# BrandonHanx/TextReID

Hardware: AMD Instinct MI355X
Metric: image-text pairs/sec (train), CLIP-RN50 + BiGRU MoCo step, bs128/GPU (higher is better)
Workload: dtype f32; 1 GPU; configs[1]: CLIP-RN50 + GRU, bs128/GPU, 384x128 images, 64-token captions, MoCo queue 8192, fp32, 1xMI355X; random-init weights, synthetic inputs resident in HBM; global_batch=128, parallelism=dp1, optimizer=Adam (fused multi-tensor), step_launch=eager launches, four streams (chosen by the probe over the recorded step)

## Files before the change

textreid_amd/csrc/gemm_p16.hip:

```cpp

#include <algorithm>
#include <mutex>
#include <type_traits>

#include "split_common.h"

namespace trid {

constexpr int P16_BK = 32;
constexpr int A_CONV_S2 = 3;

constexpr int p16_lds_bytes(int BM, int BN, int NW, int STAGES) {
    const int st = STAGES * (BM + BN) * 128;
    return (NW == 12 && BM * BN * 4 > st) ? BM * BN * 4 : st;
}

template <int N>
__device__ __forceinline__ void wait_vmcnt() {
    asm volatile("s_waitcnt vmcnt(%0)" ::"n"(N) : "memory");
}

__device__ __forceinline__ void dma16(const __amdgpu_buffer_rsrc_t& rs, uint4* lds_base, unsigned voffset, unsigned soffset) {
    typedef __attribute__((address_space(3))) void* lds_ptr;
    __builtin_amdgcn_raw_ptr_buffer_load_lds(rs, (lds_ptr)lds_base, 16, voffset, soffset, 0, 0);
}

typedef int v4i_t __attribute__((ext_vector_type(4)));
__device__ __forceinline__ v4i_t raw_rsrc(const void* base, unsigned bytes) {
    const unsigned long long b = (unsigned long long)(uintptr_t)base;
    v4i_t r;
    r[0] = __builtin_amdgcn_readfirstlane((int)(unsigned)b);
    r[1] = __builtin_amdgcn_readfirstlane((int)(unsigned)(b >> 32) & 0xffff);
    r[2] = __builtin_amdgcn_readfirstlane((int)bytes);
    r[3] = 0x00020000;
    return r;
}
__device__ __forceinline__ void dma16_asm(const v4i_t& rs, unsigned lds_byte_addr, unsigned voffset, unsigned soffset) {
    asm volatile("s_mov_b32 m0, %0\n\ts_nop 0\n\tbuffer_load_dwordx4 %1, %2, %3 offen lds" ::"s"(__builtin_amdgcn_readfirstlane(lds_byte_addr)), "v"(voffset), "s"(rs), "s"(__builtin_amdgcn_readfirstlane(soffset)) : "memory", "m0");
}

template <int AMODE, int BM, int BN, int WM, int WN, int STAGES, int PL, bool PP = false, int SP = 0>
__global__ __launch_bounds__(WM* WN * 64, (WM * WN == 4 && STAGES == 2) ? 2 : (WM * WN == 8 && (BM + BN) * 128 * STAGES <= 80 * 1024 ? 4 : ((WM * WN == 6 || WM * WN == 12) ? 3 : 2))) void gemm_p16_kernel(GemmParams p) {
    constexpr int NW = WM * WN;
    constexpr bool CONV = AMODE == A_CONV || AMODE == A_CONV_S2, S2 = AMODE == A_CONV_S2;
    constexpr int BKE = PL == 2 ? 32 : 64;
    constexpr int EB = PL == 2 ? 4 : 2;
    constexpr int TM = BM / (32 * WM), TN = BN / (32 * WN);
    constexpr int A_CH = BM / 8, B_CH = BN / 8;
    constexpr int A_PW = (A_CH + NW - 1) / NW, B_PW = (B_CH + NW - 1) / NW;
    constexpr int PER_TILE = A_PW + B_PW;
    constexpr int STAGE_SLOTS = (BM + BN) * 8;
    extern __shared__ __attribute__((aligned(16))) uint4 smem[];

    const float scaleA = (PL == 2 && p.a_amax != nullptr) ? f16_scale_of(*p.a_amax) : 1.f;
    const float scaleB = (PL == 2 && p.b_amax != nullptr) ? f16_scale_of(*p.b_amax) : 1.f;
    float ev_bound = 0.f, ev_rinv = 1.f;
    unsigned ev_seen = 0;
    if (p.c_fmt == 1) {
        ev_bound = eval_out_bound(p.ev);
        ev_rinv = p.res16 != nullptr ? 1.f / f16_scale_of(*p.res16_amax) : 1.f;
        if (p.ev.out_tmax != nullptr) ev_seen = __hip_atomic_load(reinterpret_cast<const unsigned*>(p.ev.out_tmax), __ATOMIC_RELAXED, __HIP_MEMORY_SCOPE_AGENT);
    }

    const int tid = threadIdx.x;
    const int lane = tid & 63;
    const int wave = __builtin_amdgcn_readfirstlane(tid >> 6);
    const int wm = wave / WN, wn = wave % WN;
    const int khalf = lane >> 5;

    const uint32_t nwg = (uint32_t)p.mblocks * (uint32_t)p.nblocks;
    const uint32_t lid = xcd_remap(blockIdx.x, nwg);
    const int mb = lid / p.nblocks, nb = lid % p.nblocks;
    const int m0 = mb * BM, n0 = nb * BN;
    const int z = blockIdx.z;
    const int bz = z / p.splits, sz = z % p.splits;
    const int kt_begin = sz * (p.k_chunk / BKE);
    const int kt_end = min(p.K / BKE, kt_begin + p.k_chunk / BKE);
    const int nk = kt_end - kt_begin;

    const char* A = reinterpret_cast<const char*>(p.A) + (long long)bz * p.sA * EB;
    const char* Bp = reinterpret_cast<const char*>(p.B) + (long long)bz * p.sB * EB;
    float* __restrict__ C = p.C + (long long)bz * p.sC + (long long)sz * p.sSplit;
    const float* __restrict__ bias = p.bias ? p.bias + (long long)bz * p.sBias : nullptr;

    constexpr unsigned OOB = 0x80000000u;
    const long long a_ld_bytes = (CONV ? (long long)p.Cin : p.lda) * EB;
    const long long a_rows = CONV ? (S2 ? (long long)(p.M / (p.RH * p.RW)) * p.H * p.W : (long long)p.M) + 2 * p.W + 2 : p.M;
    const char* a_base = (CONV) ? A - (long long)(p.W + 1) * a_ld_bytes : A;
    const __amdgpu_buffer_rsrc_t rsA = __builtin_amdgcn_make_buffer_rsrc((void*)a_base, 0, (unsigned)(a_rows * a_ld_bytes), 0x00020000);
    const __amdgpu_buffer_rsrc_t rsB = __builtin_amdgcn_make_buffer_rsrc((void*)Bp, 0, (unsigned)((long long)p.N * p.ldb * EB), 0x00020000);

    unsigned voA[A_PW], voB[B_PW], amask[A_PW];
#pragma unroll
    for (int j = 0; j < A_PW; ++j) {
        const int c = j * NW + wave;
        const int r = 8 * c + (lane >> 3);
        const int s = (lane & 7) ^ ((r >> 1) & 7);
        const int m = m0 + r;
        voA[j] = (c < A_CH && m < p.M) ? (unsigned)((long long)m * a_ld_bytes + 16 * s) : OOB;
        amask[j] = 0x1ffu;
        if constexpr (S2) {
            const uint32_t mm = m < p.M ? (uint32_t)m : 0u;
            const uint32_t q = fdiv(mm, p.fdW);
            const int x = (int)mm - (int)q * p.RW;
            const uint32_t b = fdiv(q, p.fdH);
            const int y = (int)q - (int)b * p.RH;
            const long long src = ((long long)b * p.H + 2 * y) * p.W + 2 * x;
            voA[j] = (c < A_CH && m < p.M) ? (unsigned)(src * a_ld_bytes + 16 * s) : OOB;
            unsigned mk = 0;
#pragma unroll
            for (int t = 0; t < 9; ++t) {
                const int yy = 2 * y + t / 3 - 1, xx = 2 * x + t % 3 - 1;
                if (yy >= 0 && yy < p.H && xx >= 0 && xx < p.W) mk |= 1u << t;
            }
            amask[j] = mk;
        } else if (CONV) {
            const uint32_t q = fdiv((uint32_t)m, p.fdW);
            const int x = m - (int)q * p.W;
            const uint32_t b = fdiv(q, p.fdH);
            const int y = (int)q - (int)b * p.H;
            unsigned mk = 0;
#pragma unroll
            for (int t = 0; t < 9; ++t) {
                const int yy = y + t / 3 - 1, xx = x + t % 3 - 1;
                if (yy >= 0 && yy < p.H && xx >= 0 && xx < p.W) mk |= 1u << t;
            }
            amask[j] = mk;
        }
    }
#pragma unroll
    for (int j = 0; j < B_PW; ++j) {
        const int c = j * NW + wave;
        const int r = 8 * c + (lane >> 3);
        const int s = (lane & 7) ^ ((r >> 1) & 7);
        const int n = n0 + r;
        voB[j] = (c < B_CH && n < p.N) ? (unsigned)((long long)n * p.ldb * EB + 16 * s) : OOB;
    }
    const int cgroups = (CONV) ? p.Cin / BKE : 1;

    const unsigned smem_base = (unsigned)(uintptr_t)(__attribute__((address_space(3))) void*)smem;
    auto issue = [&](int kt, int stage) {
        uint4* sA = smem + stage * STAGE_SLOTS;
        uint4* sB = sA + BM * 8;
        unsigned soA, soB;
        int tap = 0;
        if (CONV) {
            tap = kt % 9;
            const int cg = kt / 9;
            soA = (unsigned)((((tap / 3) * p.W + (tap % 3)) * (long long)p.Cin * EB) + cg * 128);
            soB = (unsigned)((tap * cgroups + cg) * 128);
        } else {
            soA = soB = (unsigned)(kt * 128);
        }
#pragma unroll
        for (int j = 0; j < A_PW; ++j) {
            const int c = j * NW + wave;
            if (A_CH % NW != 0 && c >= A_CH) break;
            unsigned vo = voA[j];
            if (CONV) vo = ((amask[j] >> tap) & 1u) ? vo : OOB;
            dma16(rsA, sA + c * 64, vo, soA);
        }
#pragma unroll
        for (int j = 0; j < B_PW; ++j) {
            const int c = j * NW + wave;
            if (B_CH % NW != 0 && c >= B_CH) break;
            dma16(rsB, sB + c * 64, voB[j], soB);
        }
    };

    v16f acc[TM][TN];
#pragma unroll
    for (int i = 0; i < TM; ++i)
#pragma unroll
        for (int j = 0; j < TN; ++j)
#pragma unroll
            for (int r = 0; r < 16; ++r) acc[i][j][r] = 0.f;

    const int xs = (lane >> 1) & 7;
    const int a_row = wm * (32 * TM) + (lane & 31);
    const int b_row = wn * (32 * TN) + (lane & 31);

    auto compute = [&](int stage) {
        const uint4* sA = smem + stage * STAGE_SLOTS;
        const uint4* sB = sA + BM * 8;
        if constexpr (PL == 1) {
#pragma unroll
            for (int ks = 0; ks < 4; ++ks) {
                bf16x8 a[TM], b[TN];
                const int s = (2 * ks + khalf) ^ xs;
#pragma unroll
                for (int i = 0; i < TM; ++i) a[i] = __builtin_bit_cast(bf16x8, sA[(a_row + 32 * i) * 8 + s]);
#pragma unroll
                for (int j = 0; j < TN; ++j) b[j] = __builtin_bit_cast(bf16x8, sB[(b_row + 32 * j) * 8 + s]);
#pragma unroll
                for (int i = 0; i < TM; ++i)
#pragma unroll
                    for (int j = 0; j < TN; ++j) acc[i][j] = __builtin_amdgcn_mfma_f32_32x32x16_bf16(a[i], b[j], acc[i][j], 0, 0, 0);
            }
        } else {
#pragma unroll
            for (int ks = 0; ks < 2; ++ks) {
                f16x8 a[2][TM], b[2][TN];
#pragma unroll
                for (int pl = 0; pl < 2; ++pl) {
                    const int s = (4 * pl + 2 * ks + khalf) ^ xs;
#pragma unroll
                    for (int i = 0; i < TM; ++i) a[pl][i] = __builtin_bit_cast(f16x8, sA[(a_row + 32 * i) * 8 + s]);
#pragma unroll
                    for (int j = 0; j < TN; ++j) b[pl][j] = __builtin_bit_cast(f16x8, sB[(b_row + 32 * j) * 8 + s]);
                }
#pragma unroll
                for (int i = 0; i < TM; ++i)
#pragma unroll
                    for (int j = 0; j < TN; ++j) acc[i][j] = __builtin_amdgcn_mfma_f32_32x32x16_f16(a[0][i], b[1][j], acc[i][j], 0, 0, 0);
#pragma unroll
                for (int i = 0; i < TM; ++i)
#pragma unroll
                    for (int j = 0; j < TN; ++j) acc[i][j] = __builtin_amdgcn_mfma_f32_32x32x16_f16(a[1][i], b[0][j], acc[i][j], 0, 0, 0);
#pragma unroll
                for (int i = 0; i < TM; ++i)
#pragma unroll
                    for (int j = 0; j < TN; ++j) acc[i][j] = __builtin_amdgcn_mfma_f32_32x32x16_f16(a[0][i], b[0][j], acc[i][j], 0, 0, 0);
            }
        }
    };

    if constexpr (PP) {
        static_assert(STAGES == 2 && NW % 2 == 0, "ping-pong schedule: two stages, an even number of waves");
        constexpr int NKS = PL == 2 ? 2 : 4, NPL = PL == 2 ? 2 : 1;
        uint4 fa[NKS][NPL][TM], fb[NKS][NPL][TN];
        auto rd = [&](int stage) {
            const uint4* sA = smem + stage * STAGE_SLOTS;
            const uint4* sB = sA + BM * 8;
#pragma unroll
            for (int ks = 0; ks < NKS; ++ks)
#pragma unroll
                for (int pl = 0; pl < NPL; ++pl) {
                    const int s = ((PL == 2 ? 4 * pl : 0) + 2 * ks + khalf) ^ xs;
#pragma unroll
                    for (int i = 0; i < TM; ++i) fa[ks][pl][i] = sA[(a_row + 32 * i) * 8 + s];
#pragma unroll
                    for (int j = 0; j < TN; ++j) fb[ks][pl][j] = sB[(b_row + 32 * j) * 8 + s];
                }
            asm volatile("s_waitcnt lgkmcnt(0)" ::: "memory");
        };
        auto mm = [&]() {
            __builtin_amdgcn_s_setprio(1);
#pragma unroll
            for (int ks = 0; ks < NKS; ++ks) {
                if constexpr (PL == 1) {
#pragma unroll
                    for (int i = 0; i < TM; ++i)
#pragma unroll
                        for (int j = 0; j < TN; ++j)
                            acc[i][j] = __builtin_amdgcn_mfma_f32_32x32x16_bf16(__builtin_bit_cast(bf16x8, fa[ks][0][i]), __builtin_bit_cast(bf16x8, fb[ks][0][j]), acc[i][j], 0, 0, 0);
                } else {
#pragma unroll
                    for (int i = 0; i < TM; ++i)
#pragma unroll
                        for (int j = 0; j < TN; ++j)
                            acc[i][j] = __builtin_amdgcn_mfma_f32_32x32x16_f16(__builtin_bit_cast(f16x8, fa[ks][0][i]), __builtin_bit_cast(f16x8, fb[ks][1][j]), acc[i][j], 0, 0, 0);
#pragma unroll
                    for (int i = 0; i < TM; ++i)
#pragma unroll
                        for (int j = 0; j < TN; ++j)
                            acc[i][j] = __builtin_amdgcn_mfma_f32_32x32x16_f16(__builtin_bit_cast(f16x8, fa[ks][1][i]), __builtin_bit_cast(f16x8, fb[ks][0][j]), acc[i][j], 0, 0, 0);
#pragma unroll
                    for (int i = 0; i < TM; ++i)
// ... 21 lines not shown
                bar();
            }
            bar();
        } else {
            if (1 < nk) issue(kt_begin + 1, 1);
            bar();
            for (int t = 0; t < nk; ++t) {
                rd(t & 1);
                wait_vmcnt<0>();
                bar();
                if (t + 2 < nk) issue(kt_begin + t + 2, t & 1);
                mm();
                bar();
            }
        }
    } else if constexpr (SP != 0) {
        static_assert(STAGES == 2 && PL == 2, "software pipeline: two stages, P16 operands");
        constexpr int NM = 3 * TM * TN;
        const v4i_t rsA_s = raw_rsrc(a_base, (unsigned)(a_rows * a_ld_bytes)), rsB_s = raw_rsrc(Bp, (unsigned)((long long)p.N * p.ldb * EB));
        uint4 f0a[2][TM], f0b[2][TN], f1a[2][TM], f1b[2][TN];
        auto rd = [&](int stage, int ks, uint4 (&fa)[2][TM], uint4 (&fb)[2][TN]) {
            const uint4* sA = smem + stage * STAGE_SLOTS;
            const uint4* sB = sA + BM * 8;
#pragma unroll
            for (int pl = 0; pl < 2; ++pl) {
                const int s = (4 * pl + 2 * ks + khalf) ^ xs;
#pragma unroll
                for (int i = 0; i < TM; ++i) fa[pl][i] = sA[(a_row + 32 * i) * 8 + s];
#pragma unroll
                for (int j = 0; j < TN; ++j) fb[pl][j] = sB[(b_row + 32 * j) * 8 + s];
            }
        };
        auto mm1 = [&](const uint4 (&fa)[2][TM], const uint4 (&fb)[2][TN], int idx) {
            const int pr = idx / (TM * TN), ij = idx % (TM * TN), i = ij / TN, j = ij % TN;
            const int pa = pr == 1 ? 1 : 0, pb = pr == 0 ? 1 : 0;
            acc[i][j] = __builtin_amdgcn_mfma_f32_32x32x16_f16(__builtin_bit_cast(f16x8, fa[pa][i]), __builtin_bit_cast(f16x8, fb[pb][j]), acc[i][j], 0, 0, 0);
        };
        int n_tap = 0, n_dx = 0;
        unsigned n_soA = 0, n_soB = 0, n_rowA = 0, n_cgA = 0;
        const unsigned cin_b = (unsigned)p.Cin * EB, roww_b = (unsigned)p.W * cin_b;
        {
            const int kt = kt_begin;
            if (CONV) {
                n_tap = kt % 9;
                const int cg = kt / 9;
                n_dx = n_tap % 3;
                n_rowA = (unsigned)(n_tap / 3) * roww_b;
                n_cgA = (unsigned)cg * 128u;
                n_soA = n_rowA + (unsigned)n_dx * cin_b + n_cgA;
                n_soB = (unsigned)(n_tap * cgroups + cg) * 128u;
            } else {
                n_soA = n_soB = (unsigned)kt * 128u;
            }
        }
        unsigned c_soA = 0, c_soB = 0;
        int c_tap = 0;
        auto latch = [&]() {
            c_soA = n_soA; c_soB = n_soB; c_tap = n_tap;
        };
        auto advance = [&]() {
            if (CONV) {
                ++n_tap; ++n_dx;
                n_soB += (unsigned)cgroups * 128u;
                if (n_dx == 3) { n_dx = 0; n_rowA += roww_b; }
                if (n_tap == 9) { n_tap = 0; n_rowA = 0; n_cgA += 128u; n_soB = n_soB - 9u * (unsigned)cgroups * 128u + 128u; }
                n_soA = n_rowA + (unsigned)n_dx * cin_b + n_cgA;
            } else {
                n_soA += 128u; n_soB += 128u;
            }
        };
        auto piece = [&](int stage, int q) {
            if (q < A_PW) {
                const int c = q * NW + wave;
                if (A_CH % NW != 0 && c >= A_CH) return;
                unsigned vo = voA[q];
                if (CONV) vo = ((amask[q] >> c_tap) & 1u) ? vo : OOB;
                dma16_asm(rsA_s, smem_base + (unsigned)(stage * STAGE_SLOTS + c * 64) * 16u, vo, c_soA);
            } else {
                const int j = q - A_PW, c = j * NW + wave;
                if (B_CH % NW != 0 && c >= B_CH) return;
                dma16_asm(rsB_s, smem_base + (unsigned)(stage * STAGE_SLOTS + BM * 8 + c * 64) * 16u, voB[j], c_soB);
            }
        };
        auto tile = [&](int t, auto stage_c) {
            constexpr int stage = decltype(stage_c)::value;
            const bool has_prev = t > 0, has_next = t + 1 < nk;
            asm volatile("s_waitcnt vmcnt(0)" ::: "memory");
            __builtin_amdgcn_s_waitcnt(0x0070);
            __builtin_amdgcn_s_barrier();
            asm volatile("" ::: "memory");
            rd(stage, 0, f0a, f0b);
            __builtin_amdgcn_sched_barrier(0);
            latch();
            if (has_next && ((SP & 3) == 1 || !has_prev)) {
#pragma unroll
                for (int q = 0; q < PER_TILE; ++q) piece(stage ^ 1, q);
            }
            __builtin_amdgcn_sched_barrier(0);
            if constexpr ((SP & 4) != 0) __builtin_amdgcn_s_setprio(1);
            if (has_prev) {
                int q = 0;
#pragma unroll
                for (int m = 0; m < NM; ++m) {
                    mm1(f1a, f1b, m);
                    if constexpr ((SP & 3) == 2) {
                        __builtin_amdgcn_sched_barrier(0);
#pragma unroll
                        for (int e = 0; e < PER_TILE; ++e)
                            if (e == q && q * NM < (m + 1) * PER_TILE) {
                                if (has_next) piece(stage ^ 1, q);
                                ++q;
                            }
                        __builtin_amdgcn_sched_barrier(0);
                    }
                }
            }
            __builtin_amdgcn_sched_barrier(0);
            rd(stage, 1, f1a, f1b);
            __builtin_amdgcn_sched_barrier(0);
            advance();
#pragma unroll
            for (int m = 0; m < NM; ++m) mm1(f0a, f0b, m);
            if constexpr ((SP & 4) != 0) __builtin_amdgcn_s_setprio(0);
            __builtin_amdgcn_sched_barrier(0);
        };
        typedef std::integral_constant<int, 0> S0;
        typedef std::integral_constant<int, 1> S1;
        if (nk > 0) {
            latch();
#pragma unroll
            for (int q = 0; q < PER_TILE; ++q) piece(0, q);
            advance();
            int t = 0;
            for (; t + 1 < nk; t += 2) {
                tile(t, S0());
                tile(t + 1, S1());
            }
            if (t < nk) tile(t, S0());
#pragma unroll
            for (int m = 0; m < NM; ++m) mm1(f1a, f1b, m);
        }
    } else {
#pragma unroll
        for (int s = 0; s < STAGES - 1; ++s)
            if (s < nk) issue(kt_begin + s, s);
        int stage = 0, istage = (STAGES - 1) % STAGES;
        for (int t = 0; t < nk; ++t) {
            const int ahead = min(STAGES - 2, nk - 1 - t);
            if (STAGES >= 4 && ahead == 2) wait_vmcnt<2 * PER_TILE>();
            else if (STAGES >= 3 && ahead >= 1) wait_vmcnt<PER_TILE>();
            else wait_vmcnt<0>();
            __builtin_amdgcn_s_barrier();
            asm volatile("" ::: "memory");
            if (t + STAGES - 1 < nk) issue(kt_begin + t + STAGES - 1, istage);
            compute(stage);
            stage = (stage + 1 == STAGES) ? 0 : stage + 1;
            istage = (istage + 1 == STAGES) ? 0 : istage + 1;
        }
    }

    const float unscale = 1.f / (scaleA * scaleB);
    const int row_base = m0 + wm * (32 * TM) + 4 * khalf;
    const int col_base = n0 + wn * (32 * TN) + (lane & 31);
    unsigned short* __restrict__ Cb = reinterpret_cast<unsigned short*>(p.C);

    auto emit_stats = [&]() {
        __syncthreads();
        float4* red = reinterpret_cast<float4*>(smem);
        constexpr int SR = (BM % 128 == 0) ? 128 : BM;
        constexpr int WPS = SR / (32 * TM);
        constexpr int WR = 32 * TM;
        const int slab = wm / WPS;
        const int nw_i = min(max(p.M - (m0 + wm * WR), 0), WR);
        const float inv_nw = nw_i > 0 ? 1.f / (float)nw_i : 0.f;
        const bool whole = m0 + BM <= p.M;
#pragma unroll
        for (int j = 0; j < TN; ++j) {
            const int cl = wn * (32 * TN) + 32 * j + (lane & 31);
            float s = 0.f, lo = INFINITY, hi = -INFINITY;
            if (whole) {
#pragma unroll
                for (int i = 0; i < TM; ++i)
#pragma unroll
                    for (int r = 0; r < 16; ++r) {
                        s += acc[i][j][r];
                        lo = fminf(lo, acc[i][j][r]);
                        hi = fmaxf(hi, acc[i][j][r]);
                    }
            } else {
#pragma unroll
                for (int i = 0; i < TM; ++i)
#pragma unroll
                    for (int r = 0; r < 16; ++r) {
                        const int row = row_base + i * 32 + (r & 3) + 8 * (r >> 2);
                        if (row < p.M) {
                            s += acc[i][j][r];
                            lo = fminf(lo, acc[i][j][r]);
                            hi = fmaxf(hi, acc[i][j][r]);
                        }
                    }
            }
            s += __shfl_xor(s, 32, 64);
            lo = fminf(lo, __shfl_xor(lo, 32, 64));
            hi = fmaxf(hi, __shfl_xor(hi, 32, 64));
            const float mean = s * inv_nw;
            float q = 0.f;
            if (whole) {
#pragma unroll
                for (int i = 0; i < TM; ++i)
#pragma unroll
                    for (int r = 0; r < 16; ++r) {
                        const float d = acc[i][j][r] - mean;
                        q += d * d;
                    }
            } else {
#pragma unroll
                for (int i = 0; i < TM; ++i)
#pragma unroll
                    for (int r = 0; r < 16; ++r) {
                        const int row = row_base + i * 32 + (r & 3) + 8 * (r >> 2);
                        const float d = acc[i][j][r] - mean;
                        if (row < p.M) q += d * d;
                    }
            }
            q += __shfl_xor(q, 32, 64);
            if (khalf == 0) red[wm * BN + cl] = make_float4(mean, q, lo, hi);
        }
        __syncthreads();
        if ((wm % WPS) == 0 && khalf == 0) {
#pragma unroll
            for (int j = 0; j < TN; ++j) {
                const int cl = wn * (32 * TN) + 32 * j + (lane & 31);
                const int col = n0 + cl;
                float cnt = 0.f, mean = 0.f, m2 = 0.f, lo = INFINITY, hi = -INFINITY;
#pragma unroll
                for (int w = 0; w < WPS; ++w) {
                    const int nb_i = min(max(p.M - (m0 + (slab * WPS + w) * WR), 0), WR);
                    if (nb_i > 0) {
                        const float4 v = red[(slab * WPS + w) * BN + cl];
                        const float nb = (float)nb_i, nt = cnt + nb, d = v.x - mean;
                        mean += d * (nb / nt);
// ... 586 lines not shown

__global__ __launch_bounds__(256) void p16_unpack_kernel(const uint4* __restrict__ in, long long rows, int K,
                                                         const float* __restrict__ amax, float* __restrict__ out) {
    const float inv = 1.f / (amax != nullptr ? f16_scale_of(*amax) : 1.f);
    const int K8 = K / 8;
    const long long total = rows * K8;
    for (long long idx = (long long)blockIdx.x * 256 + threadIdx.x; idx < total; idx += (long long)gridDim.x * 256) {
        const long long row = idx / K8;
        const int kg = (int)(idx - row * K8);
        const uint4* src = in + row * (K / 4) + (kg >> 2) * 8 + (kg & 3);
        const uint4 h = src[0], l = src[4];
        const unsigned hw[4] = {h.x, h.y, h.z, h.w}, lw[4] = {l.x, l.y, l.z, l.w};
        float v[8];
#pragma unroll
        for (int q = 0; q < 4; ++q) {
            const f16x2 a = __builtin_bit_cast(f16x2, hw[q]), b = __builtin_bit_cast(f16x2, lw[q]);
            v[2 * q] = ((float)a.x + (float)b.x) * inv;
            v[2 * q + 1] = ((float)a.y + (float)b.y) * inv;
        }
        float* dst = out + row * K + 8 * kg;
        *reinterpret_cast<float4*>(dst) = make_float4(v[0], v[1], v[2], v[3]);
        *reinterpret_cast<float4*>(dst + 4) = make_float4(v[4], v[5], v[6], v[7]);
    }
}

__global__ __launch_bounds__(256) void p16_pack_wt_kernel(const float* __restrict__ w, int N, int T, int C, int flip,
                                                          const float* __restrict__ amax, uint4* __restrict__ out) {
    const float scale = amax != nullptr ? f16_scale_of(*amax) : 1.f;
    const int K = T * N, K8 = K / 8;
    const long long total = (long long)C * K8;
    for (long long idx = (long long)blockIdx.x * 256 + threadIdx.x; idx < total; idx += (long long)gridDim.x * 256) {
        const int kg = (int)(idx / C);
        const int c = (int)(idx - (long long)kg * C);
        const int k0 = 8 * kg;
        const int tp = k0 / N, n0 = k0 - tp * N;
        const int t = flip ? T - 1 - tp : tp;
        float v[8];
#pragma unroll
        for (int i = 0; i < 8; ++i) v[i] = w[((long long)(n0 + i) * T + t) * C + c] * scale;
        unsigned h[4], l[4];
#pragma unroll
        for (int q = 0; q < 4; ++q) f16_split2(v[2 * q], v[2 * q + 1], h[q], l[q]);
        uint4* dst = out + (long long)c * (K / 4) + (kg >> 2) * 8 + (kg & 3);
        dst[0] = make_uint4(h[0], h[1], h[2], h[3]);
        dst[4] = make_uint4(l[0], l[1], l[2], l[3]);
    }
}

__global__ __launch_bounds__(256) void p16_pack_multi_kernel(const long long* __restrict__ table, const float* __restrict__ amax,
                                                             int transposed, int fmt) {
    const long long* e = table + 6 * (long long)blockIdx.y;
    const float* __restrict__ w = reinterpret_cast<const float*>(e[0]);
    uint4* __restrict__ out = reinterpret_cast<uint4*>(e[1]);
    const int N = (int)e[2], T = (int)e[3], C = (int)e[4];
    const float scale = fmt == 1 ? f16_scale_of(amax[e[5]]) : 1.f;
    if (!transposed) {
        const int K = T * C, K8 = K / 8;
        const long long total = (long long)N * K8;
        for (long long idx = (long long)blockIdx.x * 256 + threadIdx.x; idx < total; idx += (long long)gridDim.x * 256) {
            const long long row = idx / K8;
            const int kg = (int)(idx - row * K8);
            const float4 u = *reinterpret_cast<const float4*>(w + row * K + 8 * kg);
            const float4 v = *reinterpret_cast<const float4*>(w + row * K + 8 * kg + 4);
            const float x8[8] = {u.x, u.y, u.z, u.w, v.x, v.y, v.z, v.w};
            pack8_store(out, row, K, kg, x8, scale, fmt);
        }
    } else {
        const int K = T * N, K8 = K / 8;
        const long long total = (long long)C * K8;
        for (long long idx = (long long)blockIdx.x * 256 + threadIdx.x; idx < total; idx += (long long)gridDim.x * 256) {
            const int kg = (int)(idx / C);
            const int c = (int)(idx - (long long)kg * C);
            const int k0 = 8 * kg;
            const int tp = k0 / N, n0 = k0 - tp * N;
            const int t = T - 1 - tp;
            float v[8];
#pragma unroll
            for (int i = 0; i < 8; ++i) v[i] = w[((long long)(n0 + i) * T + t) * C + c];
            pack8_store(out, c, K, kg, v, scale, fmt);
        }
    }
}

template <int AMODE, int BM, int BN, int WM, int WN, int STAGES, int PL = 2, bool PP = false, int SP = 0>
static int launch_p16(GemmParams& p, hipStream_t stream) {
    p.mblocks = (p.M + BM - 1) / BM;
    p.nblocks = (p.N + BN - 1) / BN;
    dim3 grid((unsigned)(p.mblocks * p.nblocks), 1, (unsigned)(p.batch * p.splits));
    static const size_t pad = getenv("TRID_GEMM_LDS_PAD") ? (size_t)atoi(getenv("TRID_GEMM_LDS_PAD")) * 1024 : 0;
    const size_t lds = std::max((size_t)p16_lds_bytes(BM, BN, WM * WN, STAGES), pad);
    static std::once_flag once;
    static hipError_t attr_err = hipSuccess;
    std::call_once(once, [lds] {
        if (lds > 48 * 1024)
            attr_err = hipFuncSetAttribute((const void*)gemm_p16_kernel<AMODE, BM, BN, WM, WN, STAGES, PL, PP, SP>,
                                           hipFuncAttributeMaxDynamicSharedMemorySize, (int)lds);
    });
    if (attr_err != hipSuccess) {
        set_error("trid_gemm_p16: cannot reserve %zu B of LDS: %s", lds, hipGetErrorString(attr_err));
        return (int)attr_err;
    }
    hipLaunchKernelGGL((gemm_p16_kernel<AMODE, BM, BN, WM, WN, STAGES, PL, PP, SP>), grid, dim3(WM * WN * 64), lds, stream, p);
    return check_launch("trid_gemm_p16");
}

static bool tile192_rule(int M, int N) {
    static const int env = getenv("TRID_P16_TILE192") ? atoi(getenv("TRID_P16_TILE192")) : 0;
    if (!env || M % 192 != 0 || N % 128 != 0) return false;
    const long long t128 = (long long)((M + 127) / 128) * (N / 128), t192 = (long long)(M / 192) * (N / 128);
    return t128 > 256 && t128 < 512 && t192 % 256 == 0;
}

template <int AMODE>
static int pick_p16(GemmParams& p, int variant, int planes, hipStream_t stream) {
    if (planes == 1) {
        if (p.N <= 64) return launch_p16<AMODE, 128, 64, 2, 2, 3, 1>(p, stream);
        return launch_p16<AMODE, 128, 128, 2, 4, 2, 1>(p, stream);
    }
    if (p.N <= 32) return launch_p16<AMODE, 256, 32, 4, 1, 3>(p, stream);
    if (p.N <= 64) return launch_p16<AMODE, 128, 64, 2, 2, 3>(p, stream);
    static const int def_env = getenv("TRID_P16_DEFAULT_VARIANT") ? atoi(getenv("TRID_P16_DEFAULT_VARIANT")) : 12;
    if (variant < 0 && p.stats != nullptr && tile192_rule(p.M, p.N)) variant = 15;
    const bool tile8 = variant == 3 || variant == 10 || variant == 12 || variant == 14;
    if (variant < 0 || ((p.c_fmt == 1 || p.bb.y != nullptr) && !tile8)) variant = def_env;
    switch (variant) {
        case 1: return launch_p16<AMODE, 128, 128, 2, 2, 3>(p, stream);
        case 2: return launch_p16<AMODE, 256, 128, 4, 2, 3>(p, stream);
        case 3: return launch_p16<AMODE, 128, 128, 2, 4, 2>(p, stream);
        case 4: return launch_p16<AMODE, 256, 128, 4, 2, 2>(p, stream);
        case 5: return launch_p16<AMODE, 128, 128, 2, 4, 3>(p, stream);
        case 8: return launch_p16<AMODE, 128, 64, 2, 2, 2>(p, stream);
        case 9: return launch_p16<AMODE, 96, 128, 3, 2, 2>(p, stream);
        case 6: return launch_p16<AMODE, 128, 128, 2, 4, 2, 2, true>(p, stream);
        case 7: return launch_p16<AMODE, 256, 128, 4, 2, 2, 2, true>(p, stream);
        case 10: return launch_p16<AMODE, 128, 128, 2, 4, 2, 2, false, 1>(p, stream);
        case 11: return launch_p16<AMODE, 128, 128, 2, 2, 2, 2, false, 1>(p, stream);
        case 12: return launch_p16<AMODE, 128, 128, 2, 4, 2, 2, false, 2>(p, stream);
        case 13: return launch_p16<AMODE, 128, 128, 2, 2, 2, 2, false, 2>(p, stream);
        case 15: return launch_p16<AMODE, 192, 128, 3, 4, 2, 2, false, 2>(p, stream);
        case 16: return launch_p16<AMODE, 192, 128, 3, 4, 2, 2, false, 1>(p, stream);
        case 14: return launch_p16<AMODE, 128, 128, 2, 4, 2, 2, false, 6>(p, stream);
        default: return launch_p16<AMODE, 128, 128, 2, 2, 2>(p, stream);
    }
}

}

using namespace trid;

extern "C" int trid_p16_pack_f32(const float* x, long long rows, int K, long long ldx, const float* amax, void* out, int fmt,
                                 void* stream) {
    TRID_REQUIRE(x && out && rows > 0 && K > 0 && K % 32 == 0 && ldx % 4 == 0 && aligned16(x) && aligned16(out) && (fmt == 1 || fmt == 2),
                 "trid_p16_pack_f32: needs K %% 32 == 0, 16-byte aligned rows and fmt 1 / 2 (K=%d)", K);
    hipLaunchKernelGGL(p16_pack_kernel, dim3(grid_for(rows * (K / 8), 256, 8192)), dim3(256), 0, (hipStream_t)stream, x, rows, K,
                       ldx, amax, (uint4*)out, fmt);
    return check_launch("trid_p16_pack_f32");
}

extern "C" int trid_p16_unpack_f32(const void* in, long long rows, int K, const float* amax, float* out, void* stream) {
    TRID_REQUIRE(in && out && rows > 0 && K > 0 && K % 32 == 0 && aligned16(in) && aligned16(out), "trid_p16_unpack_f32: bad arguments");
    hipLaunchKernelGGL(p16_unpack_kernel, dim3(grid_for(rows * (K / 8), 256, 8192)), dim3(256), 0, (hipStream_t)stream,
                       (const uint4*)in, rows, K, amax, out);
    return check_launch("trid_p16_unpack_f32");
}

extern "C" int trid_p16_pack_wt_f32(const float* w, int N, int T, int C, int flip, const float* amax, void* out, void* stream) {
    TRID_REQUIRE(w && out && N > 0 && T > 0 && C > 0 && N % 8 == 0 && (T * N) % 32 == 0 && aligned16(out),
                 "trid_p16_pack_wt_f32: needs N %% 8 == 0 and T*N %% 32 == 0 (N=%d T=%d)", N, T);
    hipLaunchKernelGGL(p16_pack_wt_kernel, dim3(grid_for((long long)C * (T * N / 8), 256, 8192)), dim3(256), 0, (hipStream_t)stream,
                       w, N, T, C, flip, amax, (uint4*)out);
    return check_launch("trid_p16_pack_wt_f32");
}

template <int BMODE, int BM, int PL, int SP = 0>
static int launch_p16_wgrad(GemmParams& p, hipStream_t stream) {
    constexpr int STAGES = 2;
    p.mblocks = (p.M + BM - 1) / BM;
    p.nblocks = (p.N + 127) / 128;
    static const int xcd_env = getenv("TRID_WGRAD_XCD") ? atoi(getenv("TRID_WGRAD_XCD")) : 1;
    p.xcd_split = (xcd_env && p.splits >= 8) ? 1 : 0;
    dim3 grid((unsigned)(p.mblocks * p.nblocks), 1, (unsigned)p.splits);
    if (p.xcd_split) grid = dim3((unsigned)(p.mblocks * p.nblocks) * 8u * (unsigned)((p.splits + 7) / 8), 1, 1);
    static const size_t pad = getenv("TRID_WGRAD_LDS_PAD") ? (size_t)atoi(getenv("TRID_WGRAD_LDS_PAD")) * 1024 : 0;
    const size_t lds = std::max((size_t)STAGES * ((BM / 32) + 4) * 4096, pad);
    static std::once_flag once;
    static hipError_t attr_err = hipSuccess;
    std::call_once(once, [lds] {
        if (lds > 48 * 1024)
            attr_err = hipFuncSetAttribute((const void*)gemm_p16_wgrad_kernel<BMODE, BM, STAGES, PL, SP>, hipFuncAttributeMaxDynamicSharedMemorySize, (int)lds);
    });
    if (attr_err != hipSuccess) {
        set_error("trid_gemm_p16_wgrad: cannot reserve %zu B of LDS: %s", lds, hipGetErrorString(attr_err));
        return (int)attr_err;
    }
    hipLaunchKernelGGL((gemm_p16_wgrad_kernel<BMODE, BM, STAGES, PL, SP>), grid, dim3(512), lds, stream, p);
    return check_launch("trid_gemm_p16_wgrad");
}

extern "C" int trid_gemm_p16_wgrad(const trid_gemm_desc* d, void* stream_) {
    hipStream_t stream = (hipStream_t)stream_;
    TRID_REQUIRE(d != nullptr && d->A && d->B && d->C, "trid_gemm_p16_wgrad: null operand");
    TRID_REQUIRE(d->a_mode == A_MC && (d->b_mode == B_NC || d->b_mode == B_CONV), "trid_gemm_p16_wgrad: loader modes A_MC x B_NC / B_CONV only");
    TRID_REQUIRE(d->conv_stride != 2, "trid_gemm_p16_wgrad: the stride-2 gather is a trid_gemm_f32 loader");
    const int planes = d->precision == 1 ? 1 : 2;
    const int gc = planes == 1 ? 64 : 32;
    TRID_REQUIRE(d->M > 0 && d->N > 0 && d->K > 0 && d->M % gc == 0 && d->N % gc == 0 && d->lda % gc == 0,
                 "trid_gemm_p16_wgrad: M, N and the row pitches must be multiples of %d (M=%d N=%d)", gc, d->M, d->N);
    TRID_REQUIRE(d->batch == 1 && d->splits >= 1 && !d->accumulate && !d->bias && !d->residual && !d->relu && !d->stats,
                 "trid_gemm_p16_wgrad: plain or split-K output only");
    TRID_REQUIRE(aligned16(d->A) && aligned16(d->B) && aligned16(d->C), "trid_gemm_p16_wgrad: operands must be 16-byte aligned");
    GemmParams p;
    memset(&p, 0, sizeof(p));
    p.A = d->A; p.B = d->B; p.C = d->C;
    p.M = d->M; p.N = d->N; p.K = d->K;
    p.lda = d->lda; p.ldb = d->ldb; p.ldc = d->ldc;
    p.batch = 1; p.splits = d->splits;
    p.alpha = d->alpha;
    p.H = d->H; p.W = d->W; p.Cin = d->Cin;
    p.a_amax = d->a_amax; p.b_amax = d->b_amax;
    if (d->b_mode == B_CONV) {
        TRID_REQUIRE(d->H > 0 && d->W > 0 && d->Cin > 0 && d->Cin % gc == 0 && d->N == 9 * d->Cin && d->K % (d->H * d->W) == 0,
                     "trid_gemm_p16_wgrad: B_CONV needs Cin %% %d == 0, N == 9*Cin, K a multiple of H*W", gc);
        p.fdW = make_fastdiv((uint32_t)d->W);
        p.fdH = make_fastdiv((uint32_t)d->H);
// ... 165 lines not shown
```

textreid_amd/ops.py:

```python

import ctypes
import os
import math

import torch

from . import lib as L
from .lib import GemmDesc, call

A_KC, A_MC, A_CONV = L.TRID_A_KC, L.TRID_A_MC, L.TRID_A_CONV
B_KC, B_NC, B_CONV = L.TRID_B_KC, L.TRID_B_NC, L.TRID_B_CONV

BN_EPS = 1e-5
BN_MOMENTUM = 0.1
STATS_ROWS = 128
GEMM_PRECISION = int(__import__("os").environ.get("TRID_GEMM_PRECISION", "6"))
CONV_PRECISION = int(__import__("os").environ.get("TRID_CONV_PRECISION", "16"))


def conv_precision():
    return CONV_PRECISION if GEMM_PRECISION == 6 else GEMM_PRECISION


_raw_stream = torch._C._cuda_getCurrentRawStream
# ... 399 lines not shown
        raise RuntimeError("stem_conv1_wgrad: a contiguous [B,3,H,W] image batch and a contiguous fp32 [B,Ho,Wo,32] gradient are needed")
    dw = empty((32, 3, 3, 3), images)
    slabs = empty((_query("trid_stem_conv1_wgrad_slabs"), 32 * 27), images)
    call("trid_stem_conv1_wgrad_f32", _p(images), _p(dy), _p(dw), _p(slabs), Bi, Hi, Wi, stream())
    return dw


def bn_finalize_minmax(partials, M, gamma, beta, running_mean, running_var, relu, bound, momentum=BN_MOMENTUM, eps=BN_EPS, rows_per_part=STATS_ROWS):
    C = gamma.numel()
    st = BNState(C, gamma)
    if isinstance(partials, Partials):
        partials, rows_per_part = partials.data, partials.rows
    call("trid_bn_finalize_minmax_f32", _p(partials), partials.shape[0], rows_per_part, M, C, _p(gamma), _p(beta),
         _p(running_mean), _p(running_var), momentum, eps, _p(st.mean), _p(st.invstd), _p(st.scale), _p(st.shift),
         1 if relu else 0, _p(bound), _p(bn_finalize_ws(partials.device)), stream())
    if running_mean is not None:
        note_parameter_write()
    return st


def bn_apply_p16(y, st, bound, relu=True, res=None, res_st=None, bound_res=None, want_mask=False, fmt=1):
    C = y.shape[-1]
    M = y.numel() // C
    out = p16_empty(y.shape, y, fmt)
    mask = torch.empty(((M * C // 4 + 63) // 64) * 4, dtype=torch.int64, device=y.device) if want_mask else None
    res_p16 = isinstance(res, P16)
    osum = amax_slot(y.device) if (res is not None and fmt == 1) else None
    res_fmt = res.fmt if res_p16 else (2 if (res is not None and res.dtype == torch.bfloat16) else 0)
    call("trid_bn_apply_p16_f32", _p(y), 2 if y.dtype == torch.bfloat16 else 0, _p(st.scale), _p(st.shift),
         _p(res.data if res_p16 else res), _p(res_st.scale) if res_st else None, _p(res_st.shift) if res_st else None, res_fmt,
         _p(res.amax) if res_p16 else None, _p(out), fmt, M, C, 1 if relu else 0, _p(mask), _p(bound), _p(bound_res), _p(osum),
         stream())
    o = P16(out, (osum if res is not None else bound) if fmt == 1 else None, fmt)
    return (o, mask) if want_mask else o


USE_EVAL_P16 = os.environ.get("TRID_EVAL_P16", "1") != "0"


def eval_bound_coefs(entries, device):
    rows = [[w.data_ptr(), w.shape[0], w.numel() // w.shape[0], sc.data_ptr(), sh.data_ptr()] for (w, sc, sh) in entries]
    table = torch.tensor(rows, dtype=torch.int64, device=device)
    coef = torch.zeros(len(rows), 2, dtype=torch.float32, device=device)
    call("trid_eval_bound_coefs_f32", _p(table), len(rows), _p(coef), stream())
    return coef


def bn_eval_bound(partials, st, relu):
    bound = amax_slot(partials.data.device)
    call("trid_bn_eval_bound_f32", _p(partials.data), partials.data.shape[0], partials.data.shape[1], _p(st.scale), _p(st.shift),
         1 if relu else 0, _p(bound), stream())
    return bound


def conv3x3_halo_eval_pool_ok(H, W, Cin, Cout):
    return bool(_query("trid_conv3x3_halo_eval_pool_ok", int(H), int(W), int(Cin), int(Cout)))


def conv3x3_halo_eval_p16(x, w, st, coef, relu=True, pool=False):
    Bi, H, W, C = x.shape
    N = w.shape[0]
    out = p16_empty((Bi, H // 2, W // 2, N) if pool else (Bi, H, W, N), x.data, 1)
    bound, tmax = amax_slot(x.data.device), amax_slot(x.data.device)
    call("trid_conv3x3_halo_eval_p16", _p(x.data), _p(x.amax), _p(w.data), _p(w.amax), _p(st.scale), _p(st.shift), _p(out), _p(coef), _p(x.tmax),
         _p(bound), _p(tmax), Bi, H, W, C, N, 1 if relu else 0, 1 if pool else 0, stream())
    return P16(out, bound, 1, tmax)


def stem_conv1_eval_p16(images, w, st, coef, img_amax, relu=True):
    Bi, Cin, Hi, Wi = images.shape
    if Cin != 3 or w.shape[0] != 32 or not w.is_contiguous() or not images.is_contiguous():
        raise RuntimeError("stem_conv1_eval_p16: a contiguous [B,3,H,W] image batch and contiguous [32,3,3,3] filters are needed")
    out = p16_empty((Bi, (Hi + 1) // 2, (Wi + 1) // 2, 32), images, 1)
    bound, tmax = amax_slot(images.device), amax_slot(images.device)
    call("trid_stem_conv1_eval_p16", _p(images), _p(w), _p(st.scale), _p(st.shift), _p(out), _p(coef), _p(img_amax), _p(bound), _p(tmax),
         Bi, Hi, Wi, 1 if relu else 0, stream())
    return P16(out, bound, 1, tmax)


def conv_eval_pool_ok(H, W, N):
    return W % 2 == 0 and H % 2 == 0 and 128 % W == 0 and (128 // W) % 2 == 0 and (H * W) % 128 == 0 and N > 64


def conv_eval_p16(x, w, st, coef, relu=True, res=None, conv3=False, pool=False):
    C = x.shape[-1]
    M = x.data.numel() // C
    N = w.shape[0]
    K = 9 * C if conv3 else C
    shape = tuple(x.shape[:-1]) + (N,)
    if pool:
        assert conv3 and res is None and conv_eval_pool_ok(x.shape[1], x.shape[2], N)
        shape = (x.shape[0], x.shape[1] // 2, x.shape[2] // 2, N)
    out = p16_empty(shape, x.data, 1)
    dev = x.data.device
    if conv3 and res is None and not pool and USE_HALO_BLOCKS and conv3x3_halo_rows(x.shape[1], x.shape[2], C, N):
        return conv3x3_halo_eval_p16(x, w, st, coef, relu)
    bound, tmax = amax_slot(dev), amax_slot(dev)
    if not conv3 and USE_STREAM and K in (64, 128, 256) and _query("trid_conv1x1_bn_res_p16_ok", int(M), int(N), int(K)):
        call("trid_conv1x1_eval_p16", _p(x.data), _p(x.amax), _p(w.data), _p(w.amax), _p(st.scale), _p(st.shift),
             _p(res.data) if res is not None else None, _p(res.amax) if res is not None else None, _p(out), _p(coef), _p(x.tmax),
             _p(res.tmax) if res is not None else None, _p(bound), _p(tmax), M, N, K, 1 if relu else 0, stream())
        return P16(out, bound, 1, tmax)
    d = GemmDesc()
    d.A, d.B, d.C = _p(x.data), _p(w.data), _p(out)
    d.M, d.N, d.K = M, N, K
    d.lda, d.ldb, d.ldc = C, K, N
    d.batch, d.splits = 1, 1
    d.a_mode, d.b_mode = (A_CONV if conv3 else A_KC), B_KC
    d.alpha = 1.0
    if conv3:
        d.H, d.W, d.Cin = x.shape[1], x.shape[2], C
    d.precision = 16
    d.a_amax, d.b_amax = _p(x.amax), _p(w.amax)
    d.relu = 1 if relu else 0
    d.c_format = 1
    d.col_scale, d.bias = _p(st.scale), _p(st.shift)
    if res is not None:
        d.res_p16, d.res_amax, d.eval_tres = _p(res.data), _p(res.amax), _p(res.tmax)
    d.eval_coef, d.eval_tin = _p(coef), _p(x.tmax)
    d.out_bound, d.out_tmax = _p(bound), _p(tmax)
    d.eval_pool_w = x.shape[2] if pool else 0
    call("trid_gemm_p16", ctypes.addressof(d), -1, stream())
    return P16(out, bound, 1, tmax)


USE_FUSED_EXPAND = __import__("os").environ.get("TRID_FUSED_EXPAND", "1") != "0"


def conv1x1_bn_res_ok(M, N, K):
    return USE_FUSED_EXPAND and USE_STREAM and K <= 128 and bool(_query("trid_conv1x1_bn_res_p16_ok", int(M), int(N), int(K)))


def conv1x1_stats_p16(x, w):
    C = x.shape[-1]
    M = x.data.numel() // C
    N = w.shape[0]
    rows = _query("trid_gemm_p16_stream_stats_rows", int(M), int(N), int(C))
    st = empty(((M + rows - 1) // rows, N, 4), x.data)
    call("trid_gemm_p16_stream", _p(x.data), _p(x.amax), _p(w.data), _p(w.amax), None, N, _p(st), M, N, C, 0, None, stream())
    return Partials(st, rows)


def conv1x1_bn_res_p16(x, w, st, bound, res, relu=True, want_mask=False, keep_y=False):
    C = x.shape[-1]
    M = x.data.numel() // C
    N = w.shape[0]
    shape = tuple(x.shape[:-1]) + (N,)
    out = p16_empty(shape, x.data, 1)
    y = empty(shape, x.data) if keep_y else None
    mask = torch.empty(((M * N // 4 + 63) // 64) * 4, dtype=torch.int64, device=x.data.device) if want_mask else None
    osum = amax_slot(x.data.device)
    call("trid_conv1x1_bn_res_p16", _p(x.data), _p(x.amax), _p(w.data), _p(w.amax), _p(y), _p(st.scale), _p(st.shift), _p(res.data), _p(res.amax),
         _p(out), _p(bound), _p(res.amax), _p(osum), _p(mask), M, N, C, 1 if relu else 0, stream())
    return P16(out, osum, 1), mask, y


def bn_apply_pool2_p16(y, st, bound, relu=True, fmt=1):
    src = y.data if isinstance(y, P16) else y
    Bi, H, W, C = src.shape
    out = p16_empty((Bi, H // 2, W // 2, C), src, fmt)
    call("trid_bn_apply_pool2_p16_f32", _p(src), _p(st.scale) if st else None, _p(st.shift) if st else None,
         y.fmt if isinstance(y, P16) else (2 if y.dtype == torch.bfloat16 else 0), _p(y.amax) if isinstance(y, P16) else None, _p(out), fmt, Bi, H, W, C,
         1 if (relu and st is not None) else 0, _p(bound), stream())
    return P16(out, bound if fmt == 1 else None, fmt, y.tmax if (isinstance(y, P16) and st is None and fmt == 1) else None)


def bn_bwd_p16(g, y, st, mask_mode, act=None, pooled=False, want_dres=False, fmt=1, presummed=None):
    Bi, H, W, C = y.shape
    dg = empty((2, C), y)
    dgamma, dbeta = dg[0], dg[1]
    bound = None
    g_fmt = 2 if g.dtype == torch.bfloat16 else 0
    y_fmt = 2 if y.dtype == torch.bfloat16 else 0
    if presummed is not None:
        assert fmt == 1 and g_fmt == 0 and y_fmt == 0 and not pooled and presummed.y is y
        assert (mask_mode == 3 and presummed.mask is act) if presummed.mask is not None else mask_mode == (1 if presummed.relu else 0)
        bound = amax_slot(y.device)
        call("trid_bn_bwd_final_f32", _p(presummed.ws), _p(presummed.ws2), presummed.M, C, _p(st.scale), _p(dgamma), _p(dbeta), _p(bound), stream())
    elif fmt == 1:
        ws = _bn_ws(C, y)
        assert g_fmt == 0 and y_fmt == 0
        bound = amax_slot(y.device)
        call("trid_bn_bwd_reduce_bound_f32", _p(g), _p(y), _p(act), _p(st.mean), _p(st.invstd), _p(st.scale), _p(st.shift),
             mask_mode, 1 if pooled else 0, Bi, H, W, C, _p(dgamma), _p(dbeta), _p(ws), _p(bound), stream())
    else:
        ws = _bn_ws(C, y)
        call("trid_bn_bwd_reduce_g_f32", _p(g), g_fmt, _p(y), y_fmt, _p(act), _p(st.mean), _p(st.invstd), _p(st.scale), _p(st.shift),
             mask_mode, 1 if pooled else 0, Bi, H, W, C, _p(dgamma), _p(dbeta), _p(ws), stream())
    dy = p16_empty(y.shape, y, fmt)
    dres = torch.empty(y.shape, dtype=g.dtype, device=y.device) if want_dres else None
    call("trid_bn_bwd_apply_p16_f32", _p(g), g_fmt, _p(y), y_fmt, _p(act), _p(st.mean), _p(st.invstd), _p(st.scale), _p(st.shift),
         _p(dgamma), _p(dbeta), mask_mode, 1 if pooled else 0, Bi, H, W, C, _p(dy), fmt, _p(dres), _p(bound), stream())
    return P16(dy, bound, fmt), dgamma, dbeta, dres


USE_BN_DUAL = os.environ.get("TRID_BN_DUAL", "1") != "0"


def bn_bwd_dual_ok(g, y1, y2, fmt=1):
    C = y1.shape[-1]
    CQ = C // 4
    return (USE_BN_DUAL and fmt == 1 and g.dtype == torch.float32 and y1.dtype == torch.float32 and y2.dtype == torch.float32 and g.is_contiguous()
            and tuple(y1.shape) == tuple(y2.shape) == tuple(g.shape) and C % 32 == 0 and (256 % CQ == 0 or CQ % 256 == 0))


# ... 487 lines not shown
```

Before: 3171 pairs/s.

## Add 16x16x32 MFMA path to P16 GEMM as default for large K

Adds an MFMA-shape template parameter to the P16 GEMM kernel. When it is set, each 32x32 output block is computed as four 16x16x32 f16 MFMA blocks with a permuted A-row mapping, and a permlane16 swap at the end restores the 32x32 accumulator layout. A new software-pipelined tile loop splits the A-fragment reads. Variants 17 and 18 use this path, and the default variant now becomes 17 when K is at least 512. The aim is better MFMA throughput or LDS read scheduling for deep-K GEMMs, at the cost of extra register pressure, more LDS reads and an epilogue shuffle.

```diff
diff --git a/textreid_amd/csrc/gemm_p16.hip b/textreid_amd/csrc/gemm_p16.hip
--- a/textreid_amd/csrc/gemm_p16.hip
+++ b/textreid_amd/csrc/gemm_p16.hip
@@ -9,6 +9,7 @@
 
 constexpr int P16_BK = 32;
 constexpr int A_CONV_S2 = 3;
+constexpr int P16_MFMA16_MIN_K = 512, P16_MFMA16_VARIANT = 17;
 
 constexpr int p16_lds_bytes(int BM, int BN, int NW, int STAGES) {
     const int st = STAGES * (BM + BN) * 128;
@@ -39,7 +40,7 @@
     asm volatile("s_mov_b32 m0, %0\n\ts_nop 0\n\tbuffer_load_dwordx4 %1, %2, %3 offen lds" ::"s"(__builtin_amdgcn_readfirstlane(lds_byte_addr)), "v"(voffset), "s"(rs), "s"(__builtin_amdgcn_readfirstlane(soffset)) : "memory", "m0");
 }
 
-template <int AMODE, int BM, int BN, int WM, int WN, int STAGES, int PL, bool PP = false, int SP = 0>
+template <int AMODE, int BM, int BN, int WM, int WN, int STAGES, int PL, bool PP = false, int SP = 0, int MS = 0>
 __global__ __launch_bounds__(WM* WN * 64, (WM * WN == 4 && STAGES == 2) ? 2 : (WM * WN == 8 && (BM + BN) * 128 * STAGES <= 80 * 1024 ? 4 : ((WM * WN == 6 || WM * WN == 12) ? 3 : 2))) void gemm_p16_kernel(GemmParams p) {
     constexpr int NW = WM * WN;
     constexpr bool CONV = AMODE == A_CONV || AMODE == A_CONV_S2, S2 = AMODE == A_CONV_S2;
@@ -180,10 +181,57 @@
     const int a_row = wm * (32 * TM) + (lane & 31);
     const int b_row = wn * (32 * TN) + (lane & 31);
 
+    static_assert(MS == 0 || (MS == 1 && PL == 2 && !PP), "MFMA shape 1: P16 operands, the barrier-per-tile or the software-pipelined loop");
+    typedef float v4f __attribute__((ext_vector_type(4)));
+    constexpr int NBLK = MS == 1 ? 2 : 1;
+    v4f blk[TM][TN][NBLK][NBLK];
+    if constexpr (MS == 1) {
+#pragma unroll
+        for (int i = 0; i < TM; ++i)
+#pragma unroll
+            for (int j = 0; j < TN; ++j)
+#pragma unroll
+                for (int b = 0; b < 4; ++b) blk[i][j][b >> 1][b & 1] = v4f{0.f, 0.f, 0.f, 0.f};
+    }
+    const int l16 = lane & 15, q16 = lane >> 4;
+    const int a_perm = 8 * ((l16 >> 2) & 1) + 4 * (l16 >> 3) + (l16 & 3);
+    const int a_row1 = wm * (32 * TM) + a_perm, b_row1 = wn * (32 * TN) + l16;
+    const int xs1a = a_perm >> 1, xs1b = l16 >> 1;
+    auto rd1a = [&](const uint4* sA, int pl, int i, int bi) __attribute__((always_inline)) { return sA[(a_row1 + 32 * i + 16 * bi) * 8 + ((4 * pl + q16) ^ xs1a)]; };
+    auto rd1b = [&](const uint4* sB, int pl, int j, int bj) __attribute__((always_inline)) { return sB[(b_row1 + 32 * j + 16 * bj) * 8 + ((4 * pl + q16) ^ xs1b)]; };
+    constexpr int NM1 = 3 * TM * TN * 2;
+    auto mm16 = [&](const uint4 (&fa)[2][TM], const uint4 (&fb)[2][TN][2], int bi, int idx) __attribute__((always_inline)) {
+        const int pr = idx / (TM * TN * 2), r = idx % (TM * TN * 2), i = r / (TN * 2), j = (r / 2) % TN, bj = r % 2;
+        const int pa = pr == 1 ? 1 : 0, pb = pr == 0 ? 1 : 0;
+        blk[i][j][bi][bj] = __builtin_amdgcn_mfma_f32_16x16x32_f16(__builtin_bit_cast(f16x8, fa[pa][i]), __builtin_bit_cast(f16x8, fb[pb][j][bj]), blk[i][j][bi][bj], 0, 0, 0);
+    };
+
     auto compute = [&](int stage) {
         const uint4* sA = smem + stage * STAGE_SLOTS;
         const uint4* sB = sA + BM * 8;
-        if constexpr (PL == 1) {
+        if constexpr (PL == 2 && MS == 1) {
+            uint4 a0[2][TM], a1[2][TM], b[2][TN][2];
+#pragma unroll
+            for (int pl = 0; pl < 2; ++pl) {
+#pragma unroll
+                for (int i = 0; i < TM; ++i) {
+                    a0[pl][i] = rd1a(sA, pl, i, 0);
+                    a1[pl][i] = rd1a(sA, pl, i, 1);
+                }
+#pragma unroll
+                for (int j = 0; j < TN; ++j) {
+                    b[pl][j][0] = rd1b(sB, pl, j, 0);
+                    b[pl][j][1] = rd1b(sB, pl, j, 1);
+                }
+            }
+#pragma unroll
+            for (int pr = 0; pr < 3; ++pr)
+#pragma unroll
+                for (int r = 0; r < TM * TN * 2; ++r) {
+                    mm16(a0, b, 0, pr * TM * TN * 2 + r);
+                    mm16(a1, b, 1, pr * TM * TN * 2 + r);
+                }
+        } else if constexpr (PL == 1) {
 #pragma unroll
             for (int ks = 0; ks < 4; ++ks) {
                 bf16x8 a[TM], b[TN];
@@ -371,8 +419,67 @@
                 dma16_asm(rsB_s, smem_base + (unsigned)(stage * STAGE_SLOTS + BM * 8 + c * 64) * 16u, voB[j], c_soB);
             }
         };
-        auto tile = [&](int t, auto stage_c) {
+        uint4 g0a[2][TM], g1a[2][TM], gb[2][2][TN][2];
+        auto tile16 = [&](int t, auto stage_c) __attribute__((always_inline)) {
             constexpr int stage = decltype(stage_c)::value;
+            const bool has_prev = t > 0, has_next = t + 1 < nk;
+            const uint4* sA = smem + stage * STAGE_SLOTS;
+            const uint4* sB = sA + BM * 8;
+            asm volatile("s_waitcnt vmcnt(0)" ::: "memory");
+            __builtin_amdgcn_s_waitcnt(0x0070);
+            __builtin_amdgcn_s_barrier();
+            asm volatile("" ::: "memory");
+#pragma unroll
+            for (int pl = 0; pl < 2; ++pl) {
+#pragma unroll
+                for (int i = 0; i < TM; ++i) g0a[pl][i] = rd1a(sA, pl, i, 0);
+#pragma unroll
+                for (int j = 0; j < TN; ++j) {
+                    gb[stage][pl][j][0] = rd1b(sB, pl, j, 0);
+                    gb[stage][pl][j][1] = rd1b(sB, pl, j, 1);
+                }
+            }
+            __builtin_amdgcn_sched_barrier(0);
+            latch();
+            if (has_next && ((SP & 3) == 1 || !has_prev)) {
+#pragma unroll
+                for (int q = 0; q < PER_TILE; ++q) piece(stage ^ 1, q);
+            }
+            __builtin_amdgcn_sched_barrier(0);
+            if (has_prev) {
+                int q = 0;
+#pragma unroll
+                for (int m = 0; m < NM1; ++m) {
+                    mm16(g1a, gb[stage ^ 1], 1, m);
+                    if constexpr ((SP & 3) == 2) {
+                        __builtin_amdgcn_sched_barrier(0);
+#pragma unroll
+                        for (int e = 0; e < PER_TILE; ++e)
+                            if (e == q && q * NM1 < (m + 1) * PER_TILE) {
+                                if (has_next) piece(stage ^ 1, q);
+                                ++q;
+                            }
+                        __builtin_amdgcn_sched_barrier(0);
+                    }
+                }
+            }
+            __builtin_amdgcn_sched_barrier(0);
+#pragma unroll
+            for (int pl = 0; pl < 2; ++pl)
+#pragma unroll
+                for (int i = 0; i < TM; ++i) g1a[pl][i] = rd1a(sA, pl, i, 1);
+            __builtin_amdgcn_sched_barrier(0);
+            advance();
+#pragma unroll
+            for (int m = 0; m < NM1; ++m) mm16(g0a, gb[stage], 0, m);
+            __builtin_amdgcn_sched_barrier(0);
+        };
+        auto tile = [&](int t, auto stage_c) __attribute__((always_inline)) {
+            constexpr int stage = decltype(stage_c)::value;
+            if constexpr (MS == 1) {
+                tile16(t, stage_c);
+                return;
+            }
             const bool has_prev = t > 0, has_next = t + 1 < nk;
             asm volatile("s_waitcnt vmcnt(0)" ::: "memory");
             __builtin_amdgcn_s_waitcnt(0x0070);
@@ -426,8 +533,18 @@
                 tile(t + 1, S1());
             }
             if (t < nk) tile(t, S0());
-#pragma unroll
-            for (int m = 0; m < NM; ++m) mm1(f1a, f1b, m);
+            if constexpr (MS == 1) {
+                if ((nk - 1) & 1) {
+#pragma unroll
+                    for (int m = 0; m < NM1; ++m) mm16(g1a, gb[1], 1, m);
+                } else {
+#pragma unroll
+                    for (int m = 0; m < NM1; ++m) mm16(g1a, gb[0], 1, m);
+                }
+            } else {
+#pragma unroll
+                for (int m = 0; m < NM; ++m) mm1(f1a, f1b, m);
+            }
         }
     } else {
 #pragma unroll
@@ -446,6 +563,22 @@
             stage = (stage + 1 == STAGES) ? 0 : stage + 1;
             istage = (istage + 1 == STAGES) ? 0 : istage + 1;
         }
+    }
+
+    if constexpr (MS == 1) {
+#pragma unroll
+        for (int i = 0; i < TM; ++i)
+#pragma unroll
+            for (int j = 0; j < TN; ++j)
+#pragma unroll
+                for (int bi = 0; bi < 2; ++bi)
+#pragma unroll
+                    for (int jj = 0; jj < 4; ++jj) {
+                        const float x = blk[i][j][bi][0][jj], y = blk[i][j][bi][1][jj];
+                        const auto xy = __builtin_amdgcn_permlane16_swap(__float_as_uint(x), __float_as_uint(y), false, false);
+                        acc[i][j][4 * (2 * bi) + jj] = __uint_as_float(xy[0]);
+                        acc[i][j][4 * (2 * bi + 1) + jj] = __uint_as_float(xy[1]);
+                    }
     }
 
     const float unscale = 1.f / (scaleA * scaleB);
@@ -1198,7 +1331,7 @@
     }
 }
 
-template <int AMODE, int BM, int BN, int WM, int WN, int STAGES, int PL = 2, bool PP = false, int SP = 0>
+template <int AMODE, int BM, int BN, int WM, int WN, int STAGES, int PL = 2, bool PP = false, int SP = 0, int MS = 0>
 static int launch_p16(GemmParams& p, hipStream_t stream) {
     p.mblocks = (p.M + BM - 1) / BM;
     p.nblocks = (p.N + BN - 1) / BN;
@@ -1209,14 +1342,14 @@
     static hipError_t attr_err = hipSuccess;
     std::call_once(once, [lds] {
         if (lds > 48 * 1024)
-            attr_err = hipFuncSetAttribute((const void*)gemm_p16_kernel<AMODE, BM, BN, WM, WN, STAGES, PL, PP, SP>,
+            attr_err = hipFuncSetAttribute((const void*)gemm_p16_kernel<AMODE, BM, BN, WM, WN, STAGES, PL, PP, SP, MS>,
                                            hipFuncAttributeMaxDynamicSharedMemorySize, (int)lds);
     });
     if (attr_err != hipSuccess) {
         set_error("trid_gemm_p16: cannot reserve %zu B of LDS: %s", lds, hipGetErrorString(attr_err));
         return (int)attr_err;
     }
-    hipLaunchKernelGGL((gemm_p16_kernel<AMODE, BM, BN, WM, WN, STAGES, PL, PP, SP>), grid, dim3(WM * WN * 64), lds, stream, p);
+    hipLaunchKernelGGL((gemm_p16_kernel<AMODE, BM, BN, WM, WN, STAGES, PL, PP, SP, MS>), grid, dim3(WM * WN * 64), lds, stream, p);
     return check_launch("trid_gemm_p16");
 }
 
@@ -1235,9 +1368,10 @@
     }
     if (p.N <= 32) return launch_p16<AMODE, 256, 32, 4, 1, 3>(p, stream);
     if (p.N <= 64) return launch_p16<AMODE, 128, 64, 2, 2, 3>(p, stream);
-    static const int def_env = getenv("TRID_P16_DEFAULT_VARIANT") ? atoi(getenv("TRID_P16_DEFAULT_VARIANT")) : 12;
+    static const int def_set = getenv("TRID_P16_DEFAULT_VARIANT") ? atoi(getenv("TRID_P16_DEFAULT_VARIANT")) : -1;
+    const int def_env = def_set >= 0 ? def_set : (p.K >= P16_MFMA16_MIN_K ? P16_MFMA16_VARIANT : 12);
     if (variant < 0 && p.stats != nullptr && tile192_rule(p.M, p.N)) variant = 15;
-    const bool tile8 = variant == 3 || variant == 10 || variant == 12 || variant == 14;
+    const bool tile8 = variant == 3 || variant == 10 || variant == 12 || variant == 14 || variant == 17 || variant == 18;
     if (variant < 0 || ((p.c_fmt == 1 || p.bb.y != nullptr) && !tile8)) variant = def_env;
     switch (variant) {
         case 1: return launch_p16<AMODE, 128, 128, 2, 2, 3>(p, stream);
@@ -1256,6 +1390,8 @@
         case 15: return launch_p16<AMODE, 192, 128, 3, 4, 2, 2, false, 2>(p, stream);
         case 16: return launch_p16<AMODE, 192, 128, 3, 4, 2, 2, false, 1>(p, stream);
         case 14: return launch_p16<AMODE, 128, 128, 2, 4, 2, 2, false, 6>(p, stream);
+        case 17: return launch_p16<AMODE, 128, 128, 2, 4, 2, 2, false, 2, 1>(p, stream);
+        case 18: return launch_p16<AMODE, 128, 128, 2, 4, 2, 2, false, 0, 1>(p, stream);
         default: return launch_p16<AMODE, 128, 128, 2, 2, 2>(p, stream);
     }
 }
diff --git a/textreid_amd/ops.py b/textreid_amd/ops.py
--- a/textreid_amd/ops.py
+++ b/textreid_amd/ops.py
@@ -505,7 +505,7 @@
     return W % 2 == 0 and H % 2 == 0 and 128 % W == 0 and (128 // W) % 2 == 0 and (H * W) % 128 == 0 and N > 64
 
 
-def conv_eval_p16(x, w, st, coef, relu=True, res=None, conv3=False, pool=False):
+def conv_eval_p16(x, w, st, coef, relu=True, res=None, conv3=False, pool=False, variant=-1):
     C = x.shape[-1]
     M = x.data.numel() // C
     N = w.shape[0]
@@ -543,7 +543,7 @@
     d.eval_coef, d.eval_tin = _p(coef), _p(x.tmax)
     d.out_bound, d.out_tmax = _p(bound), _p(tmax)
     d.eval_pool_w = x.shape[2] if pool else 0
-    call("trid_gemm_p16", ctypes.addressof(d), -1, stream())
+    call("trid_gemm_p16", ctypes.addressof(d), int(variant), stream())
     return P16(out, bound, 1, tmax)
 
 
```

Measured after the change: 3197 pairs/s (median of 6 runs). No clear change (+0.8%).
